# hanruihua/RDA-planner

Measured on NVIDIA H100. Metric: MPC solves/sec (T=30, 20 obs, 50 ADMM iters), higher is better.
Workload: dtype f32 state / f64 su-QP interior point

## Files before the change

### rda_planner_b200/csrc/rda_kernels.cu

```cuda
#include <cuda_runtime.h>
#include <stdio.h>
#include <stdlib.h>
#include <string.h>
#include <new>
#include "rda_hd.h"
#include "cell_solver.cuh"
#include "su_solver.cuh"
#include "cell_lean.cuh"
#include "cell_lean2.cuh"
#include "cell_disc_robot.cuh"

using namespace rda;

struct SmallLayout {
  int lam, mu, z, xi, zeta, dis, coef, pref, cur_s, cur_u, ref_s, misc, hs, su, wl, slow, total;
};

struct rda_handle {
  rda_config cfg;
  rda_tunables tun;
  RobotGeom rb;
  int B, T, N, E, R;
  int sms;
  float *lam, *mu, *z, *xi, *zeta, *dis, *coef, *pref, *cur_s, *cur_u, *ref_s, *ref_speed;
  float *resi_acc, *resi_pri, *resi_dual;
  int *status, *iters, *done, *counters, *worklist, *worklist2;
  char* su_ws;
  size_t su_ws_stride;
  int lean2;
  RobotAux ra;
  ObstacleGeom<4>* ogeo;
  unsigned char* feat;
  int* worklist0;
  float* rot;
  const float *obs_A, *obs_b;
  const int *obs_kind, *obs_count;
  int obs_tv;
  float iter_threshold;
  int launches;
  int began;
  cudaStream_t side[3];
  cudaEvent_t ev_fork, ev_join[3];
  int small_mode;
  int small_max, small_ok, small_bulk;
  SmallLayout small_L;
  float su_prune;
  int extra_min;
  int split_min;
  int parts;
};

#define RDA_CUDA(x) do { cudaError_t e_ = (x); if (e_ != cudaSuccess) return (int)e_; } while (0)

namespace {

struct WarpCtx {
  __device__ __forceinline__ int lane() const { return threadIdx.x & 31; }
  __device__ __forceinline__ int nlanes() const { return 32; }
  __device__ __forceinline__ void sync() const { __syncwarp(); }
  template <typename R> __device__ __forceinline__ R sum(R x) const {
    for (int o = 16; o > 0; o >>= 1) x += __shfl_xor_sync(0xffffffffu, x, o);
    return x;
  }
  template <typename R> __device__ __forceinline__ R min(R x) const {
    for (int o = 16; o > 0; o >>= 1) { R y = __shfl_xor_sync(0xffffffffu, x, o); x = y < x ? y : x; }
    return x;
  }
  template <typename R> __device__ __forceinline__ R max(R x) const {
    for (int o = 16; o > 0; o >>= 1) { R y = __shfl_xor_sync(0xffffffffu, x, o); x = y > x ? y : x; }
    return x;
  }
};

struct DevPtrs {
  float *lam, *mu, *z, *xi, *zeta, *dis, *coef, *pref, *cur_s, *cur_u, *ref_s, *ref_speed;
  float *resi_acc, *resi_pri, *resi_dual;
  int *status, *iters, *done, *counters, *worklist, *worklist2;
  int* wl_count;
  const ObstacleGeom<4>* ogeo;
  unsigned char* feat;
  int* worklist0;
  char* su_ws;
  size_t su_ws_stride;
  const float *obs_A, *obs_b;
  const int *obs_kind, *obs_count;
  int obs_tv;
  int B, T, N, E, R;
};

__global__ void k_begin(DevPtrs d, const float* nom_s, const float* nom_u, const float* ref_s,
                        const float* ref_speed) {
  const int T = d.T;
  const int per = 3 * (T + 1);
  const int total = d.B * per;
  for (int i = blockIdx.x * blockDim.x + threadIdx.x; i < total; i += gridDim.x * blockDim.x) {
    d.cur_s[i] = nom_s[i];
    d.ref_s[i] = ref_s[i];
    int b = i / per, r = i - b * per;
    if (r < 2 * T) d.cur_u[b * 2 * T + r] = nom_u[b * 2 * T + r];
    if (r == 0) {
      d.ref_speed[b] = ref_speed[b];
      d.done[b] = 0; d.iters[b] = 0; d.status[b] = 0;
      d.resi_acc[2 * b] = 0; d.resi_acc[2 * b + 1] = 0;
      d.resi_pri[b] = 0; d.resi_dual[b] = 0;
    }
  }
}

template <typename Real>
__device__ __forceinline__ void su_instance(const DevPtrs& d, const SuParams& P, int b, SuWork<Real>& W, WarpCtx& ctx) {
  const int T = P.T, N = P.N, NT = N * T;
  const int lane = ctx.lane();
  const float* cs = d.cur_s + (size_t)b * 3 * (T + 1);
  const float* cu = d.cur_u + (size_t)b * 2 * T;
  const float* rf = d.ref_s + (size_t)b * 3 * (T + 1);
  for (int i = lane; i < 3 * (T + 1); i += 32) {
    int r = i / (T + 1), t = i - r * (T + 1);
    W.lins[3 * t + r] = cs[i];
    W.ref[3 * t + r] = rf[i];
  }
  for (int i = lane; i < 2 * T; i += 32) {
    int r = i / T, t = i - r * T;
    W.linu[2 * t + r] = cu[i];
    W.pref[2 * t + r] = d.pref[(size_t)b * 2 * T + i];
  }
  for (int t = lane; t < T; t += 32) W.d[t] = d.dis[(size_t)b * T + t];
  float* cf = d.coef + (size_t)b * 5 * NT;
  W.hx = cf; W.hy = cf + NT; W.hc = cf + 2 * NT;
  W.vref = d.ref_speed[b];
  ctx.sync();
  int iters = 0;
  int st = su_solve<Real, WarpCtx>(P, W, ctx, cf + 3 * NT, cf + 4 * NT, &iters);
  ctx.sync();
  bool ok = st != 2;
// ... 2 lines not shown
      int r = i / (T + 1), t = i - r * (T + 1);
      float v = (float)W.s[3 * t + r];
      if (!isfinite(v)) ok = false;
    }
    for (int i = lane; i < 2 * T; i += 32) {
      int r = i / T, t = i - r * T;
      if (!isfinite((float)W.u[2 * t + r])) ok = false;
    }
    ok = ctx.min((int)ok) != 0;
  }
  if (ok) {
    float* ws = d.cur_s + (size_t)b * 3 * (T + 1);
    float* wu = d.cur_u + (size_t)b * 2 * T;
    for (int i = lane; i < 3 * (T + 1); i += 32) {
      int r = i / (T + 1), t = i - r * (T + 1);
      ws[i] = (float)W.s[3 * t + r];
    }
    for (int i = lane; i < 2 * T; i += 32) {
      int r = i / T, t = i - r * T;
      wu[i] = (float)W.u[2 * t + r];
    }
    for (int t = lane; t < T; t += 32) d.dis[(size_t)b * T + t] = (float)W.d[t];
  }
  if (lane == 0) {
    d.iters[b] += 1;
    int flag = 0;
    if (st == 1) flag |= RDA_ST_SU_NOT_CONVERGED;
    if (!ok) flag |= RDA_ST_SU_NONFINITE;
    if (flag) d.status[b] |= flag;
    atomicAdd(&d.counters[3], iters);
    atomicAdd(&d.counters[4], 1);
    if (W.restarts) atomicAdd(&d.counters[5], 1);
  }
}

template <typename Real>
__global__ void __launch_bounds__(32) k_su(DevPtrs d, SuParams P) {
  extern __shared__ __align__(16) char smem[];
  const int b = blockIdx.x;
  if (b >= d.B) return;
  if (d.done[b]) return;
  WarpCtx ctx;
  SuWork<Real> W;
  su_work_layout<Real>(P.T, P.N, &W, smem, false, d.su_ws + (size_t)b * d.su_ws_stride);
  su_instance<Real>(d, P, b, W, ctx);
}

struct CellIn {
  int b, o, t, kind;
  size_t cell;
  float px, py, cp, sp, dbar, zeta, xi0, xi1;
  const float *A, *bb;
};

__device__ __forceinline__ CellIn cell_load(const DevPtrs& d, long long idx) {
  const int T = d.T, N = d.N, E = d.E, NT = N * T;
  CellIn c;
  c.b = (int)(idx / NT);
  const int rem = (int)(idx - (long long)c.b * NT);
  c.o = rem / T; c.t = rem - c.o * T;
  const float* cs = d.cur_s + (size_t)c.b * 3 * (T + 1);
  c.px = cs[c.t + 1]; c.py = cs[(T + 1) + c.t + 1];
  sincosf(cs[2 * (T + 1) + c.t], &c.sp, &c.cp);
  c.dbar = d.dis[(size_t)c.b * T + c.t];
  c.cell = (size_t)c.b * NT + (size_t)c.o * T + c.t;
  c.zeta = d.zeta[c.cell];
  const float* xi = d.xi + (size_t)c.b * 2 * NT;
  c.xi0 = xi[(size_t)c.o * T + c.t]; c.xi1 = xi[NT + (size_t)c.o * T + c.t];
  const int tc = d.obs_tv ? (c.t + 1) : 0;
  const int Tc = d.obs_tv ? (T + 1) : 1;
  const size_t ob = ((size_t)c.b * N + c.o) * Tc + tc;
  c.A = d.obs_A + ob * E * 2;
  c.bb = d.obs_b + ob * E;
  c.kind = d.obs_kind[(size_t)c.b * N + c.o];
  return c;
}

__device__ __forceinline__ void cell_store(const DevPtrs& d, const CellIn& c, const CellOut<float>& out, float* hm2,
                                           float* dual) {
  const int T = d.T, N = d.N, E = d.E, R = d.R, NT = N * T;
  float* lam = d.lam + ((size_t)c.b * N + c.o) * E * T + c.t;
  float acc = 0.f;
  for (int i = 0; i < E; ++i) {
    float nv = out.lam[i];
    float df = nv - lam[(size_t)i * T];
    acc += df * df;
    lam[(size_t)i * T] = nv;
  }
  float* mu = d.mu + ((size_t)c.b * N + c.o) * R * T + c.t;
  for (int j = 0; j < R; ++j) {
    float nv = out.mu[j];
    float df = nv - mu[(size_t)j * T];
    acc += df * df;
    mu[(size_t)j * T] = nv;
  }
  float dz = out.z - d.z[c.cell];
  acc += dz * dz;
  d.z[c.cell] = out.z;
  *dual = acc;
  d.zeta[c.cell] = out.zeta_new;
  float* xi = d.xi + (size_t)c.b * 2 * NT;
  xi[(size_t)c.o * T + c.t] = out.xi0_new;
  xi[NT + (size_t)c.o * T + c.t] = out.xi1_new;
  *hm2 = out.hm0 * out.hm0 + out.hm1 * out.hm1;
  float* cf = d.coef + (size_t)c.b * 5 * NT + (size_t)c.o * T + c.t;
  cf[0] = out.ax;
  cf[NT] = out.ay;
  cf[2 * NT] = out.c0;
  cf[3 * NT] = out.gx;
  cf[4 * NT] = out.gy;
  if (c.o == 0) {
    d.pref[(size_t)c.b * 2 * T + c.t] = c.px;
    d.pref[(size_t)c.b * 2 * T + T + c.t] = c.py;
  }
}

template <int EC, int RC, bool LISTED>
__global__ void __launch_bounds__(128, (EC <= 4 ? 6 : 3)) k_cells_fast(DevPtrs d, RobotGeom rb, float theta) {
  const int T = d.T, N = d.N, E = d.E, R = d.R;
  const int NT = N * T;
  const long long total = LISTED ? (long long)d.wl_count[2] : (long long)d.B * NT;
  const int lane = threadIdx.x & 31;
  for (long long base = (long long)blockIdx.x * blockDim.x; base < total; base += (long long)gridDim.x * blockDim.x) {
    long long idx = base + threadIdx.x;
    bool live = idx < total;
    if (LISTED && live) idx = d.worklist0[idx];
    int b = live ? (int)(idx / NT) : -1;
    float dual = 0.f;
    bool need = false;
    if (live && (d.done[b] || d.obs_count[b] == 0)) live = false;
    if (live) {
      CellIn c = cell_load(d, idx);
      float Ar[2 * EC], br[EC], lamo[EC], muo[RC];
      if (EC == 4 && E == 4) {
        const float4 a0 = __ldg(reinterpret_cast<const float4*>(c.A));
        const float4 a1 = __ldg(reinterpret_cast<const float4*>(c.A) + 1);
        const float4 b0 = __ldg(reinterpret_cast<const float4*>(c.bb));
        Ar[0] = a0.x; Ar[1] = a0.y; Ar[2] = a0.z; Ar[3] = a0.w;
        Ar[(4) % (2 * EC)] = a1.x; Ar[(5) % (2 * EC)] = a1.y; Ar[(6) % (2 * EC)] = a1.z; Ar[(7) % (2 * EC)] = a1.w;
        br[0] = b0.x; br[1 % EC] = b0.y; br[2 % EC] = b0.z; br[3 % EC] = b0.w;
      } else {
#pragma unroll
        for (int i = 0; i < EC; ++i) {
          Ar[2 * i] = (i < E) ? __ldg(c.A + 2 * i) : 0.f;
          Ar[2 * i + 1] = (i < E) ? __ldg(c.A + 2 * i + 1) : 0.f;
          br[i] = (i < E) ? __ldg(c.bb + i) : 0.f;
        }
      }
      const float* lamp = d.lam + ((size_t)c.b * N + c.o) * E * T + c.t;
      const float* mup = d.mu + ((size_t)c.b * N + c.o) * R * T + c.t;
#pragma unroll
      for (int i = 0; i < EC; ++i) lamo[i] = (i < E) ? lamp[(size_t)i * T] : 0.f;
#pragma unroll
      for (int j = 0; j < RC; ++j) muo[j] = (j < R) ? mup[(size_t)j * T] : 0.f;
      const float zo = d.z[c.cell];
      LeanOut<EC, RC> o;
      const bool ok = cell_lean<EC, RC>(rb, c.kind, EC, Ar, br, c.px, c.py, c.cp, c.sp, c.dbar, c.zeta, c.xi0,
                                        c.xi1, theta, o);
      if (d.feat) d.feat[c.cell] = (unsigned char)(ok ? o.feat : 0);
      if (ok) {
        float* lam = d.lam + ((size_t)c.b * N + c.o) * E * T + c.t;
        float acc = 0.f;
#pragma unroll
        for (int i = 0; i < EC; ++i) {
          if (i < E) {
            const float df = o.lam[i] - lamo[i];
            acc += df * df;
            lam[(size_t)i * T] = o.lam[i];
          }
        }
        float* mu = d.mu + ((size_t)c.b * N + c.o) * R * T + c.t;
#pragma unroll
        for (int j = 0; j < RC; ++j) {
          if (j < R) {
            const float df = o.mu[j] - muo[j];
            acc += df * df;
            mu[(size_t)j * T] = o.mu[j];
          }
        }
        const float dz = o.z - zo;
        acc += dz * dz;
        d.z[c.cell] = o.z;
        dual = acc;
        d.zeta[c.cell] = o.zeta_new;
        float* cf = d.coef + (size_t)c.b * 5 * NT + (size_t)c.o * T + c.t;
        cf[0] = o.ax; cf[NT] = o.ay; cf[2 * NT] = o.c0; cf[3 * NT] = o.gx; cf[4 * NT] = o.gy;
        if (c.o == 0) {
          d.pref[(size_t)c.b * 2 * T + c.t] = c.px;
          d.pref[(size_t)c.b * 2 * T + T + c.t] = c.py;
        }
      } else {
        need = true;
      }
    }
    unsigned nm = __ballot_sync(0xffffffffu, need);
    if (nm) {
      int leader = __ffs(nm) - 1, pos = 0;
      if (lane == leader) pos = atomicAdd(&d.wl_count[0], __popc(nm));
      pos = __shfl_sync(0xffffffffu, pos, leader);
      if (need) d.worklist[pos + __popc(nm & ((1u << lane) - 1))] = (int)idx;
    }
    const bool solved = live && !need;
    if (LISTED) {
      if (solved) atomicAdd(&d.resi_acc[2 * b + 1], dual);
      unsigned fastl = __ballot_sync(0xffffffffu, solved);
      if (lane == 0 && fastl) atomicAdd(&d.counters[0], __popc(fastl));
      continue;
    }
    int b0 = __shfl_sync(0xffffffffu, b, 0);
    for (int pass = 0; pass < 2; ++pass) {
      bool mine = solved && ((pass == 0) ? (b == b0) : (b != b0));
      unsigned m = __ballot_sync(0xffffffffu, mine);
      if (m == 0) continue;
      float q = mine ? dual : 0.f;
      int leader = __ffs(m) - 1;
      int bl = __shfl_sync(0xffffffffu, b, leader);
      bool uniform = __all_sync(0xffffffffu, !mine || b == bl);
      if (uniform) {
        for (int o2 = 16; o2 > 0; o2 >>= 1) q += __shfl_xor_sync(0xffffffffu, q, o2);
        if (lane == leader) atomicAdd(&d.resi_acc[2 * bl + 1], q);
      } else if (mine) {
        atomicAdd(&d.resi_acc[2 * b + 1], q);
      }
    }
    unsigned fast = __ballot_sync(0xffffffffu, solved);
    if (lane == 0 && fast) atomicAdd(&d.counters[0], __popc(fast));
  }
}

__global__ void k_obstacle_geometry(DevPtrs d, ObstacleGeom<4>* og) {
  const int i = blockIdx.x * blockDim.x + threadIdx.x;
  if (i >= d.B * d.N) return;
  ObstacleGeom<4> g;
  if (d.obs_kind[i] == RDA_OBS_POLYGON && d.E <= 4) obstacle_geometry<4>(d.E, d.obs_A + (size_t)i * d.E * 2, d.obs_b + (size_t)i * d.E, g);
  else { obstacle_geometry<4>(0, nullptr, nullptr, g); }
  og[i] = g;
}

__global__ void k_heading(DevPtrs d, float* rot) {
  const int i = blockIdx.x * blockDim.x + threadIdx.x;
  const int T = d.T;
  if (i >= d.B * T) return;
  const int b = i / T, t = i - b * T;
  float sp, cp;
  sincosf(d.cur_s[(size_t)b * 3 * (T + 1) + 2 * (T + 1) + t], &sp, &cp);
  rot[(size_t)b * 2 * T + t] = cp;
  rot[(size_t)b * 2 * T + T + t] = sp;
}

__global__ void __launch_bounds__(128, 6) k_cells_coh(DevPtrs d, RobotGeom rb, RobotAux ra, const float* __restrict__ rot,
                                                      float theta, float invT, int tiles) {
  constexpr int EC = 4, RC = 4;
  const int T = d.T, N = d.N, E = d.E, R = d.R, NT = N * T;
  const int b = blockIdx.x / tiles;
  if (d.done[b] || d.obs_count[b] == 0) return;
  const int rem = (blockIdx.x - b * tiles) * blockDim.x + threadIdx.x;
  const int lane = threadIdx.x & 31;
  const bool live = rem < NT;
  float dual = 0.f;
  bool need = false, solved = false;
  if (live) {
    int o = (int)(((float)rem + 0.5f) * invT);
    int t = rem - o * T;
    if (t < 0) { --o; t += T; } else if (t >= T) { ++o; t -= T; }
    const size_t ib = (size_t)b;
    const float* cs = d.cur_s + ib * 3 * (T + 1);
    const float* xi = d.xi + ib * 2 * NT;
    float* lamb = d.lam + ib * N * E * T;
    float* mub = d.mu + ib * N * R * T;
    float* zb = d.z + ib * NT;
    float* zetab = d.zeta + ib * NT;
    unsigned char* featb = d.feat + ib * NT;
    const float xi0 = xi[rem], xi1 = xi[NT + rem];
    const int f = featb[rem];
    int nf = -1;
    if (xi0 == 0.f && xi1 == 0.f && (f & RDA_FEAT_VALID)) {
      const float px = cs[t + 1], py = cs[(T + 1) + t + 1];
      const float cp = rot[ib * 2 * T + t], sp = rot[ib * 2 * T + T + t];
      const float dbar = d.dis[ib * T + t], zeta = zetab[rem];
      const int lo = o * E * T + t, mo = o * R * T + t;
      float lamo[EC], muo[RC];
#pragma unroll
      for (int i = 0; i < EC; ++i) lamo[i] = (i < E) ? lamb[lo + i * T] : 0.f;
#pragma unroll
      for (int j = 0; j < RC; ++j) muo[j] = (j < R) ? mub[mo + j * T] : 0.f;
      const float zo = zb[rem];
      const ObstacleGeom<4>& og = d.ogeo[ib * N + o];
      LeanOut<EC, RC> r;
      nf = cell_lean2<EC, RC>(rb, ra, og, f, px, py, cp, sp, dbar, zeta, theta, r);
      if (nf >= 0) {
        float acc = 0.f;
#pragma unroll
        for (int i = 0; i < EC; ++i) {
          if (i < E) { const float df = r.lam[i] - lamo[i]; acc += df * df; lamb[lo + i * T] = r.lam[i]; }
        }
#pragma unroll
        for (int j = 0; j < RC; ++j) {
          if (j < R) { const float df = r.mu[j] - muo[j]; acc += df * df; mub[mo + j * T] = r.mu[j]; }
        }
        const float dz = r.z - zo;
        acc += dz * dz;
        zb[rem] = r.z;
        dual = acc;
        zetab[rem] = r.zeta_new;
        float* cf = d.coef + ib * 5 * NT + rem;
        cf[0] = r.ax; cf[NT] = r.ay; cf[2 * NT] = r.c0; cf[3 * NT] = r.gx; cf[4 * NT] = r.gy;
        if (o == 0) {
          d.pref[ib * 2 * T + t] = px;
          d.pref[ib * 2 * T + T + t] = py;
        }
        if (nf != f) featb[rem] = (unsigned char)nf;
        solved = true;
      }
    }
    need = nf < 0;
  }
  const unsigned nm = __ballot_sync(0xffffffffu, need);
  if (nm) {
    const int leader = __ffs(nm) - 1;
    int pos = 0;
    if (lane == leader) pos = atomicAdd(&d.wl_count[2], __popc(nm));
    pos = __shfl_sync(0xffffffffu, pos, leader);
    if (need) d.worklist0[pos + __popc(nm & ((1u << lane) - 1))] = b * NT + rem;
  }
  const unsigned fast = __ballot_sync(0xffffffffu, solved);
  if (fast) {
    float q = dual;
    for (int o2 = 16; o2 > 0; o2 >>= 1) q += __shfl_xor_sync(0xffffffffu, q, o2);
    if (lane == 0) { atomicAdd(&d.resi_acc[2 * b + 1], q); atomicAdd(&d.counters[0], __popc(fast)); }
  }
}

struct RowsLocal { float A[2 * RDA_MAX_EDGE], b[RDA_MAX_EDGE]; };
__device__ __forceinline__ void rows_preload(const DevPtrs& d, const CellIn& c, RowsLocal& r) {
  if (d.E == 4) {
    const float4 a0 = __ldg(reinterpret_cast<const float4*>(c.A));
    const float4 a1 = __ldg(reinterpret_cast<const float4*>(c.A) + 1);
    const float4 b0 = __ldg(reinterpret_cast<const float4*>(c.bb));
    r.A[0] = a0.x; r.A[1] = a0.y; r.A[2] = a0.z; r.A[3] = a0.w; r.A[4] = a1.x; r.A[5] = a1.y; r.A[6] = a1.z; r.A[7] = a1.w;
    r.b[0] = b0.x; r.b[1] = b0.y; r.b[2] = b0.z; r.b[3] = b0.w;
  } else {
#pragma unroll
    for (int i = 0; i < RDA_MAX_EDGE; ++i) {
      const bool in = i < d.E;
      r.A[2 * i] = in ? __ldg(c.A + 2 * i) : 0.f;
      r.A[2 * i + 1] = in ? __ldg(c.A + 2 * i + 1) : 0.f;
      r.b[i] = in ? __ldg(c.bb + i) : 0.f;
    }
  }
}

__global__ void __launch_bounds__(128) k_cells_mid(DevPtrs d, RobotGeom rb, float ro2, float theta) {
  const int count = d.wl_count[0];
  const int lane = threadIdx.x & 31;
  for (int base = blockIdx.x * blockDim.x; base < count; base += gridDim.x * blockDim.x) {
    const int wi = base + threadIdx.x;
    const bool live = wi < count;
    bool need = false;
    long long idx = 0;
    if (live) {
      idx = d.worklist[wi];
      CellIn c = cell_load(d, idx);
      RowsLocal rows;
      rows_preload(d, c, rows);
      CellWork<float> w;
      cell_front<float, false>(rb, c.kind, d.E, rows.A, rows.b, c.px, c.py, c.cp, c.sp, c.dbar, c.zeta, c.xi0, c.xi1, ro2, w);
      if (w.have) {
        CellOut<float> out;
        cell_back<float>(rb, w, c.zeta, theta, out);
        float hm2 = 0.f, dual = 0.f;
        cell_store(d, c, out, &hm2, &dual);
        atomicAdd(&d.resi_acc[2 * c.b], hm2);
        atomicAdd(&d.resi_acc[2 * c.b + 1], dual);
      } else {
        need = true;
      }
    }
    unsigned m = __ballot_sync(0xffffffffu, need);
    if (m) {
      int leader = __ffs(m) - 1, pos = 0;
      if (lane == leader) pos = atomicAdd(&d.wl_count[1], __popc(m));
      pos = __shfl_sync(0xffffffffu, pos, leader);
      if (need) d.worklist2[pos + __popc(m & ((1u << lane) - 1))] = (int)idx;
    }
    unsigned solved = __ballot_sync(0xffffffffu, live && !need);
    if (lane == 0 && solved) atomicAdd(&d.counters[0], __popc(solved));
  }
}

__global__ void __launch_bounds__(128) k_cells_dr(DevPtrs d, RobotGeom rb, float ro2, float theta) {
  const int NT = d.N * d.T;
  const long long total = (long long)d.B * NT;
  const int lane = threadIdx.x & 31;
  for (long long base = (long long)blockIdx.x * blockDim.x; base < total; base += (long long)gridDim.x * blockDim.x) {
    const long long idx = base + threadIdx.x;
    bool live = idx < total;
    const int b = live ? (int)(idx / NT) : -1;
    if (live && (d.done[b] || d.obs_count[b] == 0)) live = false;
    bool need = false;
    if (live) {
      CellIn c = cell_load(d, idx);
      CellWork<float> w;
      cell_front_dr<float>(rb, c.kind, d.E, c.A, c.bb, c.px, c.py, c.cp, c.sp, c.dbar, c.zeta, c.xi0, c.xi1, ro2, w, false);
      if (w.have) {
        CellOut<float> out;
        cell_back_dr<float>(rb, w, c.zeta, theta, out);
        float hm2 = 0.f, dual = 0.f;
        cell_store(d, c, out, &hm2, &dual);
        atomicAdd(&d.resi_acc[2 * c.b], hm2);
        atomicAdd(&d.resi_acc[2 * c.b + 1], dual);
      } else {
        need = true;
      }
    }
    const unsigned m = __ballot_sync(0xffffffffu, need);
    if (m) {
      int leader = __ffs(m) - 1, pos = 0;
      if (lane == leader) pos = atomicAdd(&d.wl_count[1], __popc(m));
      pos = __shfl_sync(0xffffffffu, pos, leader);
      if (need) d.worklist2[pos + __popc(m & ((1u << lane) - 1))] = (int)idx;
    }
    const unsigned solved = __ballot_sync(0xffffffffu, live && !need);
    if (lane == 0 && solved) atomicAdd(&d.counters[0], __popc(solved));
  }
}

__global__ void __launch_bounds__(128) k_cells_dr_mid(DevPtrs d, RobotGeom rb, float ro2, float theta) {
  const int count = d.wl_count[1];
  const int lane = threadIdx.x & 31;
  for (int base = blockIdx.x * blockDim.x; base < count; base += gridDim.x * blockDim.x) {
    const int wi = base + threadIdx.x;
    bool need = false;
    int idx = 0;
    if (wi < count) {
      idx = d.worklist2[wi];
      CellIn c = cell_load(d, idx);
      CellWork<float> w;
// ... 13 lines not shown
    const unsigned m = __ballot_sync(0xffffffffu, need);
    if (m) {
      int leader = __ffs(m) - 1, pos = 0;
      if (lane == leader) pos = atomicAdd(&d.wl_count[4], __popc(m));
      pos = __shfl_sync(0xffffffffu, pos, leader);
      if (need) d.worklist[pos + __popc(m & ((1u << lane) - 1))] = idx;
    }
  }
}

constexpr int COOP_WARPS = 4;

__global__ void __launch_bounds__(32 * COOP_WARPS) k_cells_dr_slow_coop(DevPtrs d, RobotGeom rb, float ro2, float theta) {
  __shared__ DiscSlowStore store[COOP_WARPS];
  const int count = d.wl_count[4];
  const int warp = threadIdx.x >> 5, lane = threadIdx.x & 31;
  DiscSlowStore& S = store[warp];
  WarpCtx ctx;
  for (int wi = blockIdx.x * COOP_WARPS + warp; wi < count; wi += gridDim.x * COOP_WARPS) {
    const long long idx = d.worklist[wi];
    CellIn c;
    CellWork<float> w;
    w.have = false;
    if (lane == 0) {
      c = cell_load(d, idx);
      cell_front_dr<float>(rb, c.kind, d.E, c.A, c.bb, c.px, c.py, c.cp, c.sp, c.dbar, c.zeta, c.xi0, c.xi1, ro2, w, false);
    }
    const int have = __shfl_sync(0xffffffffu, (int)w.have, 0);
    if (!have) {
      __syncwarp();
      cell_slow_dr<float, WarpCtx>(rb, w, S, ctx);
      __syncwarp();
    }
    if (lane == 0) {
      CellOut<float> out;
      cell_back_dr<float>(rb, w, c.zeta, theta, out);
      float hm2 = 0.f, dual = 0.f;
      if (out.path == CELL_FAILED) {
        dual = INFINITY;
        atomicOr(&d.status[c.b], RDA_ST_CELL_FALLBACK);
      } else {
        cell_store(d, c, out, &hm2, &dual);
      }
      atomicAdd(&d.resi_acc[2 * c.b], hm2);
      atomicAdd(&d.resi_acc[2 * c.b + 1], dual);
      atomicAdd(&d.counters[out.path == CELL_FAILED ? 2 : 1], 1);
    }
    __syncwarp();
  }
}

__global__ void __launch_bounds__(128) k_cells_extra(DevPtrs d, RobotGeom rb, float ro2, float theta) {
  const int count = d.wl_count[1];
  const int lane = threadIdx.x & 31;
  for (int base = blockIdx.x * blockDim.x; base < count; base += gridDim.x * blockDim.x) {
    const int wi = base + threadIdx.x;
    bool need = false;
    int idx = 0;
    if (wi < count) {
      idx = d.worklist2[wi];
      CellIn c = cell_load(d, idx);
      RowsLocal rows;
      rows_preload(d, c, rows);
      CellWork<float> w;
      cell_front<float, false, true>(rb, c.kind, d.E, rows.A, rows.b, c.px, c.py, c.cp, c.sp, c.dbar, c.zeta, c.xi0, c.xi1, ro2, w);
      if (w.have) {
        CellOut<float> out;
        cell_back<float>(rb, w, c.zeta, theta, out);
        float hm2 = 0.f, dual = 0.f;
        cell_store(d, c, out, &hm2, &dual);
        atomicAdd(&d.resi_acc[2 * c.b], hm2);
        atomicAdd(&d.resi_acc[2 * c.b + 1], dual);
        atomicAdd(&d.counters[1], 1);
      } else {
        need = true;
      }
    }
    const unsigned m = __ballot_sync(0xffffffffu, need);
    if (m) {
      int leader = __ffs(m) - 1, pos = 0;
      if (lane == leader) pos = atomicAdd(&d.wl_count[4], __popc(m));
      pos = __shfl_sync(0xffffffffu, pos, leader);
      if (need) d.worklist[pos + __popc(m & ((1u << lane) - 1))] = idx;
    }
  }
}

__global__ void __launch_bounds__(32 * COOP_WARPS) k_cells_slow_coop(DevPtrs d, RobotGeom rb, float ro2, float theta, int from_extra) {
  __shared__ CellSlowStore store[COOP_WARPS];
  const int count = from_extra ? d.wl_count[4] : d.wl_count[1];
  const int* list = from_extra ? d.worklist : d.worklist2;
  const int warp = threadIdx.x >> 5, lane = threadIdx.x & 31;
  CellSlowStore& S = store[warp];
  WarpCtx ctx;
  for (int wi = blockIdx.x * COOP_WARPS + warp; wi < count; wi += gridDim.x * COOP_WARPS) {
    const long long idx = list[wi];
    CellIn c;
    CellWork<float> w;
    w.have = false;
    if (lane == 0) {
      c = cell_load(d, idx);
      cell_front<float, false, true>(rb, c.kind, d.E, c.A, c.bb, c.px, c.py, c.cp, c.sp, c.dbar, c.zeta, c.xi0, c.xi1, ro2, w);
    }
    const int have = __shfl_sync(0xffffffffu, (int)w.have, 0);
    if (!have) {
      __syncwarp();
      cell_slow<float, WarpCtx>(rb, w, S, ctx);
      __syncwarp();
    }
    if (lane == 0) {
      CellOut<float> out;
      cell_back<float>(rb, w, c.zeta, theta, out);
      float hm2 = 0.f, dual = 0.f;
      if (out.path == CELL_FAILED) {
        dual = INFINITY;
        atomicOr(&d.status[c.b], RDA_ST_CELL_FALLBACK);
      } else {
        cell_store(d, c, out, &hm2, &dual);
      }
      atomicAdd(&d.resi_acc[2 * c.b], hm2);
      atomicAdd(&d.resi_acc[2 * c.b + 1], dual);
      atomicAdd(&d.counters[out.path == CELL_FAILED ? 2 : 1], 1);
    }
    __syncwarp();
  }
}

__device__ __forceinline__ void finalize_instance(const DevPtrs& d, const RobotGeom& rb, float thr, int b) {
  const int T = d.T, N = d.N, NT = N * T, R = d.R;
  float pri = 0.f, dual = 0.f;
  if (N > 0 && d.obs_count[b] != 0) {
    pri = sqrtf(d.resi_acc[2 * b]);
    dual = d.resi_acc[2 * b + 1] / (float)N;
  } else if (N > 0) {
    int o = N - 1;
    float* cf = d.coef + (size_t)b * 5 * NT + (size_t)o * T;
    for (int t = 0; t < T; ++t) {
      const float* mu = d.mu + ((size_t)b * N + o) * R * T + t;
      float muh = 0.f;
      for (int j = 0; j < R; ++j) muh += mu[(size_t)j * T] * rb.h[j];
      size_t cell = (size_t)b * NT + (size_t)o * T + t;
      cf[t] = 0.f; cf[NT + t] = 0.f;
      cf[2 * NT + t] = -muh - d.z[cell] + d.zeta[cell];
    }
  }
  d.resi_acc[2 * b] = 0.f; d.resi_acc[2 * b + 1] = 0.f;
  d.resi_pri[b] = pri; d.resi_dual[b] = dual;
  if (dual < thr && pri < thr) { d.done[b] = 1; d.status[b] |= RDA_ST_EARLY_STOP; }
}

__global__ void k_finalize(DevPtrs d, RobotGeom rb, float thr) {
  int b = blockIdx.x * blockDim.x + threadIdx.x;
  if (b == 0) { d.wl_count[0] = 0; d.wl_count[1] = 0; d.wl_count[2] = 0; d.wl_count[3] = 0; d.wl_count[4] = 0; }
  if (b >= d.B) return;
  if (d.done[b]) return;
  finalize_instance(d, rb, thr, b);
}

static SmallLayout small_layout(int T, int N, int E, int R, size_t su_bytes, size_t su_gbytes) {
  SmallLayout L;
  size_t o = 0;
  auto take = [&](size_t bytes) { o = (o + 15) & ~(size_t)15; size_t r = o; o += bytes; return (int)r; };
  const size_t NT = (size_t)N * T;
  L.lam = take(4 * N * E * T); L.mu = take(4 * N * R * T); L.z = take(4 * NT); L.xi = take(8 * NT); L.zeta = take(4 * NT);
  L.dis = take(4 * T); L.coef = take(20 * NT); L.pref = take(8 * T); L.cur_s = take(12 * (T + 1)); L.cur_u = take(8 * T);
  L.ref_s = take(12 * (T + 1)); L.misc = take(128); L.hs = take(su_gbytes); L.su = take(su_bytes);
  L.wl = take(4 * (NT + 1)); L.slow = take(4 * sizeof(CellSlowStore));
  L.total = (int)((o + 15) & ~(size_t)15);
  return L;
}

// ... 189 lines not shown
    ((float*)out.resi_pri)[b] = misc[2]; ((float*)out.resi_dual)[b] = misc[3];
    ((int*)out.status)[b] = ds.status[0]; ((int*)out.iters)[b] = ds.iters[0];
  }
}

__global__ void k_finish(DevPtrs d, rda_outputs o) {
  const int T = d.T;
  const int per = 3 * (T + 1);
  const int total = d.B * per;
  for (int i = blockIdx.x * blockDim.x + threadIdx.x; i < total; i += gridDim.x * blockDim.x) {
    o.s_opt[i] = d.cur_s[i];
    int b = i / per, r = i - b * per;
    if (r < 2 * T) o.u_opt[b * 2 * T + r] = d.cur_u[b * 2 * T + r];
    if (r == 0) {
      o.resi_pri[b] = d.resi_pri[b]; o.resi_dual[b] = d.resi_dual[b];
      o.status[b] = d.status[b]; o.iters[b] = d.iters[b];
    }
  }
}

__global__ void k_reset(DevPtrs d, RobotGeom rb) {
  const int T = d.T, N = d.N, NT = N * T, R = d.R;
  const long long total = (long long)d.B * NT;
  for (long long idx = (long long)blockIdx.x * blockDim.x + threadIdx.x; idx < total; idx += (long long)gridDim.x * blockDim.x) {
    int b = (int)(idx / NT);
    int rem = (int)(idx - (long long)b * NT);
    int o = rem / T, t = rem - o * T;
    const float* mu = d.mu + ((size_t)b * N + o) * R * T + t;
    float muh = 0.f;
    for (int j = 0; j < R; ++j) muh += mu[(size_t)j * T] * rb.h[j];
    float* cf = d.coef + (size_t)b * 5 * NT + rem;
    cf[0] = 0.f; cf[NT] = 0.f;
    cf[2 * NT] = -muh - d.z[idx] + d.zeta[idx];
  }
}

__global__ void k_fill(float* p, float v, size_t n) {
  for (size_t i = (size_t)blockIdx.x * blockDim.x + threadIdx.x; i < n; i += (size_t)gridDim.x * blockDim.x) p[i] = v;
}

DevPtrs dev_ptrs(const rda_handle* h, int b0, int nb, int part) {
  DevPtrs d;
  const size_t o = (size_t)b0, T = h->T, N = h->N, E = h->E, R = h->R, NT = N * T;
  const size_t Tc = h->obs_tv ? T + 1 : 1;
  d.lam = h->lam + o * N * E * T; d.mu = h->mu + o * N * R * T; d.z = h->z + o * NT; d.xi = h->xi + o * 2 * NT;
  d.zeta = h->zeta + o * NT; d.dis = h->dis + o * T; d.coef = h->coef + o * 5 * NT; d.pref = h->pref + o * 2 * T;
  d.cur_s = h->cur_s + o * 3 * (T + 1); d.cur_u = h->cur_u + o * 2 * T; d.ref_s = h->ref_s + o * 3 * (T + 1);
  d.ref_speed = h->ref_speed + o; d.resi_acc = h->resi_acc + 2 * o; d.resi_pri = h->resi_pri + o;
  d.resi_dual = h->resi_dual + o;
  d.status = h->status + o; d.iters = h->iters + o; d.done = h->done + o;
  d.counters = h->counters; d.wl_count = h->counters + 8 + 8 * part;
  d.ogeo = h->ogeo ? h->ogeo + o * N : nullptr;
  d.feat = h->feat ? h->feat + o * NT : nullptr;
  d.worklist0 = h->worklist0 ? h->worklist0 + o * NT : nullptr;
  d.worklist = h->worklist + o * NT; d.worklist2 = h->worklist2 + o * NT;
  d.su_ws = h->su_ws + o * h->su_ws_stride; d.su_ws_stride = h->su_ws_stride;
  d.obs_A = h->obs_A ? h->obs_A + o * N * Tc * E * 2 : nullptr;
  d.obs_b = h->obs_b ? h->obs_b + o * N * Tc * E : nullptr;
  d.obs_kind = h->obs_kind ? h->obs_kind + o * N : nullptr;
  d.obs_count = h->obs_count ? h->obs_count + o : nullptr;
  d.obs_tv = h->obs_tv;
  d.B = nb; d.T = h->T; d.N = h->N; d.E = h->E; d.R = h->R;
  return d;
}

DevPtrs dev_ptrs(const rda_handle* h) { return dev_ptrs(h, 0, h->B, 0); }

SuParams su_params(const rda_handle* h) {
  SuParams P;
  P.T = h->T; P.N = h->N; P.dynamics = h->cfg.dynamics; P.accelerated = h->cfg.accelerated;
  P.dt = h->cfg.step_time; P.L = h->cfg.wheelbase;
  P.umax[0] = h->cfg.max_speed[0]; P.umax[1] = h->cfg.max_speed[1];
  P.ab[0] = h->cfg.acce_bound[0]; P.ab[1] = h->cfg.acce_bound[1];
  P.ws = h->cfg.ws; P.wu = h->cfg.wu;
  P.slack_gain = h->tun.slack_gain; P.dmin = h->tun.min_sd; P.dmax = h->tun.max_sd;
  P.ro1 = h->tun.ro1; P.ro2 = h->tun.ro2;
  P.max_iter = 40;
  P.mu0 = 1.0f;
  P.prune = h->su_prune;
  return P;
}

int grid_for(long long n, int block, int sms) {
  long long g = (n + block - 1) / block;
  const long long cap = 16LL * sms;
  if (g > cap) g = cap;
  if (g < 1) g = 1;
  return (int)g;
}

}

extern "C" {

const char* rda_version(void) { return "rda_b200 0.1 (sm_90a)"; }

int rda_create(const rda_config* cfg, const rda_tunables* tun, rda_handle** out) {
  if (!cfg || !tun || !out) return RDA_E_ARG;
  if (cfg->batch < 1 || cfg->receding < 1 || cfg->max_obs_num < 0) return RDA_E_ARG;
  if (cfg->max_edge_num < 3 || cfg->max_edge_num > RDA_MAX_EDGE) return RDA_E_UNSUPPORTED;
  if (cfg->dynamics < 0 || cfg->dynamics > 2) return RDA_E_ARG;
  rda_handle* h = new (std::nothrow) rda_handle();
  if (!h) return RDA_E_NOMEM;
  memset(h, 0, sizeof(*h));
  h->cfg = *cfg; h->tun = *tun;
  int rc = robot_geom_from_halfspaces(cfg->G, cfg->h, cfg->robot_edges, &h->rb, cfg->robot_cone);
  if (rc) { delete h; return rc; }
  h->B = cfg->batch; h->T = cfg->receding; h->N = cfg->max_obs_num; h->E = cfg->max_edge_num;
  h->R = cfg->robot_edges;
  const size_t B = h->B, T = h->T, N = h->N, E = h->E, R = h->R, NT = N * T;
  {
    size_t g = 0;
    const size_t sm = cfg->su_fp64 ? su_work_bytes<double>((int)T, (int)N, false, &g) : su_work_bytes<float>((int)T, (int)N, false, &g);
    if (sm > 227 * 1024) { delete h; return RDA_E_UNSUPPORTED; }
    h->su_ws_stride = (g + 127) & ~(size_t)127;
  }
  int dev = 0;
  cudaError_t e = cudaGetDevice(&dev);
  if (e == cudaSuccess) e = cudaDeviceGetAttribute(&h->sms, cudaDevAttrMultiProcessorCount, dev);
  if (e != cudaSuccess) { delete h; return (int)e; }
  auto alloc = [&](float** p, size_t n) { if (e == cudaSuccess) e = cudaMalloc((void**)p, (n ? n : 1) * sizeof(float)); };
  alloc(&h->lam, B * N * E * T); alloc(&h->mu, B * N * R * T); alloc(&h->z, B * NT);
  alloc(&h->xi, B * 2 * NT); alloc(&h->zeta, B * NT); alloc(&h->dis, B * T);
  alloc(&h->coef, B * 5 * NT); alloc(&h->pref, B * 2 * T); alloc(&h->cur_s, B * 3 * (T + 1));
  alloc(&h->cur_u, B * 2 * T); alloc(&h->ref_s, B * 3 * (T + 1)); alloc(&h->ref_speed, B);
  alloc(&h->resi_acc, B * 2); alloc(&h->resi_pri, B); alloc(&h->resi_dual, B);
  alloc((float**)&h->status, B); alloc((float**)&h->iters, B); alloc((float**)&h->done, B);
  alloc((float**)&h->counters, 64);
  alloc((float**)&h->worklist, B * NT);
  alloc((float**)&h->worklist2, B * NT);
  alloc((float**)&h->su_ws, B * (h->su_ws_stride / 4));
  if (e != cudaSuccess) { rda_destroy(h); return (int)e; }
  e = cfg->su_fp64 ? cudaFuncSetAttribute(k_su<double>, cudaFuncAttributeMaxDynamicSharedMemorySize, 227 * 1024)
                   : cudaFuncSetAttribute(k_su<float>, cudaFuncAttributeMaxDynamicSharedMemorySize, 227 * 1024);
  if (e != cudaSuccess) { rda_destroy(h); return (int)e; }
  e = cudaEventCreateWithFlags(&h->ev_fork, cudaEventDisableTiming);
  for (int p = 0; p < 3; ++p) {
    if (e == cudaSuccess) e = cudaStreamCreateWithFlags(&h->side[p], cudaStreamNonBlocking);
    if (e == cudaSuccess) e = cudaEventCreateWithFlags(&h->ev_join[p], cudaEventDisableTiming);
  }
  if (e != cudaSuccess) { rda_destroy(h); return (int)e; }
  h->lean2 = h->B >= 8192 && h->E <= 4 && h->R <= 4 && h->N > 0 && !h->rb.disc;
  if (const char* l2 = getenv("RDA_B200_LEAN2")) h->lean2 = atoi(l2) != 0 && h->E <= 4 && h->R <= 4 && h->N > 0 && !h->rb.disc;
  if (h->lean2) {
    robot_aux_from_geom(h->rb, &h->ra);
    e = cudaMalloc((void**)&h->ogeo, B * N * sizeof(ObstacleGeom<4>));
    if (e == cudaSuccess) e = cudaMalloc((void**)&h->feat, B * NT ? B * NT : 1);
    if (e == cudaSuccess) e = cudaMalloc((void**)&h->worklist0, (B * NT ? B * NT : 1) * sizeof(int));
    if (e == cudaSuccess) e = cudaMalloc((void**)&h->rot, B * 2 * T * sizeof(float));
    if (e != cudaSuccess) { rda_destroy(h); return (int)e; }
  }
  h->split_min = 2048;
  h->parts = 2;
  h->su_prune = 0.5f;
  {
    size_t g = 0;
    const size_t sub = cfg->su_fp64 ? su_work_bytes<double>((int)T, (int)N, false, &g) : su_work_bytes<float>((int)T, (int)N, false, &g);
    h->small_L = small_layout((int)T, (int)N, (int)E, (int)R, sub, g);
    h->small_ok = h->small_L.total <= 200 * 1024 && !h->rb.disc;
    h->small_mode = -1; h->small_max = 2 * h->sms;
    h->small_bulk = (N > 0) && ((N * E * T) % 4 == 0) && ((N * R * T) % 4 == 0) && ((N * T) % 4 == 0);
    if (const char* v = getenv("RDA_B200_SMALL_BULK")) { if (atoi(v) == 0) h->small_bulk = 0; }
    if (const char* v = getenv("RDA_B200_SMALL")) { int x = atoi(v); if (x >= -1 && x <= 1) h->small_mode = x; }
    if (const char* v = getenv("RDA_B200_SMALL_MAX")) { int x = atoi(v); if (x >= 1) h->small_max = x; }
    if (h->small_ok) {
      if (cfg->su_fp64) e = cudaFuncSetAttribute(k_admm_small<double>, cudaFuncAttributeMaxDynamicSharedMemorySize, h->small_L.total);
      else e = cudaFuncSetAttribute(k_admm_small<float>, cudaFuncAttributeMaxDynamicSharedMemorySize, h->small_L.total);
      if (e != cudaSuccess) { rda_destroy(h); return (int)e; }
    }
  }
  if (const char* v = getenv("RDA_B200_SU_PRUNE")) { float x = (float)atof(v); if (x >= 0.f) h->su_prune = x; }
  h->extra_min = 3000;
  if (const char* v = getenv("RDA_B200_EXTRA_MIN")) { int x = atoi(v); if (x >= 1) h->extra_min = x; }
  if (const char* sm = getenv("RDA_B200_SPLIT_MIN")) { int v = atoi(sm); if (v >= 2) h->split_min = v; }
  if (const char* sp = getenv("RDA_B200_SPLIT_PARTS")) { int v = atoi(sp); if (v >= 1 && v <= 4) h->parts = v; }
  rc = rda_cold_start(h, nullptr);
  if (rc) { rda_destroy(h); return rc; }
  e = cudaDeviceSynchronize();
  if (e != cudaSuccess) { rda_destroy(h); return (int)e; }
  *out = h;
  return 0;
}

int rda_destroy(rda_handle* h) {
  if (!h) return RDA_E_ARG;
  float* bufs[] = {h->lam, h->mu, h->z, h->xi, h->zeta, h->dis, h->coef, h->pref, h->cur_s, h->cur_u,
                   h->ref_s, h->ref_speed, h->resi_acc, h->resi_pri, h->resi_dual, (float*)h->status,
                   (float*)h->iters, (float*)h->done, (float*)h->counters, (float*)h->worklist, (float*)h->worklist2, (float*)h->su_ws};
  for (float* p : bufs) if (p) cudaFree(p);
  if (h->ogeo) cudaFree(h->ogeo);
  if (h->feat) cudaFree(h->feat);
  if (h->worklist0) cudaFree(h->worklist0);
  if (h->rot) cudaFree(h->rot);
  if (h->ev_fork) cudaEventDestroy(h->ev_fork);
  for (int p = 0; p < 3; ++p) {
    if (h->ev_join[p]) cudaEventDestroy(h->ev_join[p]);
    if (h->side[p]) cudaStreamDestroy(h->side[p]);
  }
  delete h;
  return 0;
}

int rda_set_tunables(rda_handle* h, const rda_tunables* tun) {
  if (!h || !tun) return RDA_E_ARG;
  h->tun = *tun;
  return 0;
}

int rda_get_tunables(const rda_handle* h, rda_tunables* tun) {
  if (!h || !tun) return RDA_E_ARG;
  *tun = h->tun;
  return 0;
}

int rda_cold_start(rda_handle* h, void* stream) {
  if (!h) return RDA_E_ARG;
  cudaStream_t s = (cudaStream_t)stream;
  const size_t B = h->B, T = h->T, N = h->N, E = h->E, R = h->R, NT = N * T;
  RDA_CUDA(cudaMemsetAsync(h->lam, 0, B * N * E * T * 4, s));
  RDA_CUDA(cudaMemsetAsync(h->mu, 0, B * N * R * T * 4, s));
  RDA_CUDA(cudaMemsetAsync(h->z, 0, B * NT * 4, s));
  RDA_CUDA(cudaMemsetAsync(h->xi, 0, B * 2 * NT * 4, s));
  RDA_CUDA(cudaMemsetAsync(h->zeta, 0, B * NT * 4, s));
  RDA_CUDA(cudaMemsetAsync(h->coef, 0, B * 5 * NT * 4, s));
  RDA_CUDA(cudaMemsetAsync(h->pref, 0, B * 2 * T * 4, s));
  RDA_CUDA(cudaMemsetAsync(h->cur_s, 0, B * 3 * (T + 1) * 4, s));
  RDA_CUDA(cudaMemsetAsync(h->cur_u, 0, B * 2 * T * 4, s));
  RDA_CUDA(cudaMemsetAsync(h->resi_acc, 0, B * 2 * 4, s));
  RDA_CUDA(cudaMemsetAsync(h->resi_pri, 0, B * 4, s));
  RDA_CUDA(cudaMemsetAsync(h->resi_dual, 0, B * 4, s));
  RDA_CUDA(cudaMemsetAsync(h->status, 0, B * 4, s));
  RDA_CUDA(cudaMemsetAsync(h->iters, 0, B * 4, s));
  RDA_CUDA(cudaMemsetAsync(h->done, 0, B * 4, s));
  RDA_CUDA(cudaMemsetAsync(h->counters, 0, 64 * 4, s));
  if (h->feat) RDA_CUDA(cudaMemsetAsync(h->feat, 0, B * NT, s));
  k_fill<<<grid_for((long long)(B * T), 256, h->sms), 256, 0, s>>>(h->dis, 1.0f, B * T);
  RDA_CUDA(cudaGetLastError());
  h->launches = 1;
  return 0;
}

int rda_reset(rda_handle* h, void* stream) {
  if (!h) return RDA_E_ARG;
  if (h->N == 0) return 0;
  DevPtrs d = dev_ptrs(h);
// ... 236 lines not shown
```

Baseline: 25010.

## Replace index worklists with packed 80-byte cell records carrying state and duals

Worklists between the cell kernels (lean2 to fast, fast to slow, slow to extra, extra to coop) now hold full per-cell records. Each record carries position, rotation, dbar, zeta, xi and the previous lam/mu/z, so downstream kernels skip the scattered gathers and recomputation in cell_load and use the stored previous duals for the dual residual. The cost is wider worklist writes (80 bytes instead of 4 per entry), the lean2 kernel now loading duals for every cell, and two large record buffers allocated per handle.

```diff
diff --git a/rda_planner_b200/csrc/rda_kernels.cu b/rda_planner_b200/csrc/rda_kernels.cu
--- a/rda_planner_b200/csrc/rda_kernels.cu
+++ b/rda_planner_b200/csrc/rda_kernels.cu
@@ -16,6 +16,14 @@
   int lam, mu, z, xi, zeta, dis, coef, pref, cur_s, cur_u, ref_s, misc, hs, su, wl, slow, total;
 };
 
+struct __align__(16) CellRec {
+  int cell, kind;
+  float px, py, cp, sp, dbar, zeta, xi0, xi1;
+  float lam[4], mu[4], z;
+  int pad_;
+};
+static_assert(sizeof(CellRec) == 80, "CellRec: five 16-byte words");
+
 struct rda_handle {
   rda_config cfg;
   rda_tunables tun;
@@ -25,13 +33,13 @@
   float *lam, *mu, *z, *xi, *zeta, *dis, *coef, *pref, *cur_s, *cur_u, *ref_s, *ref_speed;
   float *resi_acc, *resi_pri, *resi_dual;
   int *status, *iters, *done, *counters, *worklist, *worklist2;
+  CellRec *rec_a, *rec_b;
   char* su_ws;
   size_t su_ws_stride;
   int lean2;
   RobotAux ra;
   ObstacleGeom<4>* ogeo;
   unsigned char* feat;
-  int* worklist0;
   float* rot;
   const float *obs_A, *obs_b;
   const int *obs_kind, *obs_count;
@@ -79,7 +87,7 @@
   int* wl_count;
   const ObstacleGeom<4>* ogeo;
   unsigned char* feat;
-  int* worklist0;
+  CellRec *rec_a, *rec_b;
   char* su_ws;
   size_t su_ws_stride;
   const float *obs_A, *obs_b;
@@ -188,6 +196,14 @@
   float px, py, cp, sp, dbar, zeta, xi0, xi1;
   const float *A, *bb;
 };
+
+__device__ __forceinline__ void cell_rows(const DevPtrs& d, CellIn& c) {
+  const int tc = d.obs_tv ? (c.t + 1) : 0;
+  const int Tc = d.obs_tv ? (d.T + 1) : 1;
+  const size_t ob = ((size_t)c.b * d.N + c.o) * Tc + tc;
+  c.A = d.obs_A + ob * d.E * 2;
+  c.bb = d.obs_b + ob * d.E;
+}
 
 __device__ __forceinline__ CellIn cell_load(const DevPtrs& d, long long idx) {
   const int T = d.T, N = d.N, E = d.E, NT = N * T;
@@ -212,25 +228,75 @@
   return c;
 }
 
+__device__ __forceinline__ bool rec_duals(const DevPtrs& d) { return d.E <= 4 && d.R <= 4; }
+
+__device__ __forceinline__ CellRec cell_rec(const CellIn& c) {
+  CellRec r;
+  r.cell = (int)c.cell; r.kind = c.kind;
+  r.px = c.px; r.py = c.py; r.cp = c.cp; r.sp = c.sp; r.dbar = c.dbar; r.zeta = c.zeta; r.xi0 = c.xi0; r.xi1 = c.xi1;
+  r.pad_ = 0;
+  return r;
+}
+
+__device__ __forceinline__ CellIn cell_from_rec(const DevPtrs& d, const CellRec& r) {
+  const int T = d.T, NT = d.N * T;
+  CellIn c;
+  c.cell = (size_t)r.cell;
+  c.b = r.cell / NT;
+  const int rem = r.cell - c.b * NT;
+  c.o = rem / T; c.t = rem - c.o * T;
+  c.kind = r.kind;
+  c.px = r.px; c.py = r.py; c.cp = r.cp; c.sp = r.sp; c.dbar = r.dbar; c.zeta = r.zeta; c.xi0 = r.xi0; c.xi1 = r.xi1;
+  cell_rows(d, c);
+  return c;
+}
+
+__device__ __forceinline__ CellRec cell_rec_load(const DevPtrs& d, long long idx) {
+  const CellIn c = cell_load(d, idx);
+  CellRec r = cell_rec(c);
+  const int T = d.T, N = d.N, E = d.E, R = d.R;
+  const float* lam = d.lam + ((size_t)c.b * N + c.o) * E * T + c.t;
+  const float* mu = d.mu + ((size_t)c.b * N + c.o) * R * T + c.t;
+#pragma unroll
+  for (int i = 0; i < 4; ++i) {
+    r.lam[i] = i < E ? lam[(size_t)i * T] : 0.f;
+    r.mu[i] = i < R ? mu[(size_t)i * T] : 0.f;
+  }
+  r.z = d.z[c.cell];
+  return r;
+}
+
+__device__ __forceinline__ CellRec* rec_slot(bool need, CellRec* list, int* count) {
+  const int lane = threadIdx.x & 31;
+  const unsigned m = __ballot_sync(0xffffffffu, need);
+  if (!m) return nullptr;
+  const int leader = __ffs(m) - 1;
+  int pos = 0;
+  if (lane == leader) pos = atomicAdd(count, __popc(m));
+  pos = __shfl_sync(0xffffffffu, pos, leader);
+  return need ? list + pos + __popc(m & ((1u << lane) - 1)) : nullptr;
+}
+
 __device__ __forceinline__ void cell_store(const DevPtrs& d, const CellIn& c, const CellOut<float>& out, float* hm2,
-                                           float* dual) {
+                                           float* dual, const CellRec* prev = nullptr) {
   const int T = d.T, N = d.N, E = d.E, R = d.R, NT = N * T;
+  const bool pr = prev != nullptr && rec_duals(d);
   float* lam = d.lam + ((size_t)c.b * N + c.o) * E * T + c.t;
   float acc = 0.f;
   for (int i = 0; i < E; ++i) {
     float nv = out.lam[i];
-    float df = nv - lam[(size_t)i * T];
+    float df = nv - (pr ? prev->lam[i] : lam[(size_t)i * T]);
     acc += df * df;
     lam[(size_t)i * T] = nv;
   }
   float* mu = d.mu + ((size_t)c.b * N + c.o) * R * T + c.t;
   for (int j = 0; j < R; ++j) {
     float nv = out.mu[j];
-    float df = nv - mu[(size_t)j * T];
+    float df = nv - (pr ? prev->mu[j] : mu[(size_t)j * T]);
     acc += df * df;
     mu[(size_t)j * T] = nv;
   }
-  float dz = out.z - d.z[c.cell];
+  float dz = out.z - (prev != nullptr ? prev->z : d.z[c.cell]);
   acc += dz * dz;
   d.z[c.cell] = out.z;
   *dual = acc;
@@ -258,15 +324,17 @@
   const long long total = LISTED ? (long long)d.wl_count[2] : (long long)d.B * NT;
   const int lane = threadIdx.x & 31;
   for (long long base = (long long)blockIdx.x * blockDim.x; base < total; base += (long long)gridDim.x * blockDim.x) {
-    long long idx = base + threadIdx.x;
+    const long long wi = base + threadIdx.x;
+    long long idx = wi;
     bool live = idx < total;
-    if (LISTED && live) idx = d.worklist0[idx];
+    CellRec rec;
+    if (LISTED && live) { rec = d.rec_a[wi]; idx = rec.cell; }
     int b = live ? (int)(idx / NT) : -1;
     float dual = 0.f;
     bool need = false;
-    if (live && (d.done[b] || d.obs_count[b] == 0)) live = false;
+    if (!LISTED && live && (d.done[b] || d.obs_count[b] == 0)) live = false;
     if (live) {
-      CellIn c = cell_load(d, idx);
+      CellIn c = LISTED ? cell_from_rec(d, rec) : cell_load(d, idx);
       float Ar[2 * EC], br[EC], lamo[EC], muo[RC];
       if (EC == 4 && E == 4) {
         const float4 a0 = __ldg(reinterpret_cast<const float4*>(c.A));
@@ -283,13 +351,22 @@
           br[i] = (i < E) ? __ldg(c.bb + i) : 0.f;
         }
       }
-      const float* lamp = d.lam + ((size_t)c.b * N + c.o) * E * T + c.t;
-      const float* mup = d.mu + ((size_t)c.b * N + c.o) * R * T + c.t;
+      float zo;
+      if (LISTED) {
 #pragma unroll
-      for (int i = 0; i < EC; ++i) lamo[i] = (i < E) ? lamp[(size_t)i * T] : 0.f;
+        for (int i = 0; i < EC; ++i) lamo[i] = (i < E) ? rec.lam[i % 4] : 0.f;
 #pragma unroll
-      for (int j = 0; j < RC; ++j) muo[j] = (j < R) ? mup[(size_t)j * T] : 0.f;
-      const float zo = d.z[c.cell];
+        for (int j = 0; j < RC; ++j) muo[j] = (j < R) ? rec.mu[j % 4] : 0.f;
+        zo = rec.z;
+      } else {
+        const float* lamp = d.lam + ((size_t)c.b * N + c.o) * E * T + c.t;
+        const float* mup = d.mu + ((size_t)c.b * N + c.o) * R * T + c.t;
+#pragma unroll
+        for (int i = 0; i < EC; ++i) lamo[i] = (i < E) ? lamp[(size_t)i * T] : 0.f;
+#pragma unroll
+        for (int j = 0; j < RC; ++j) muo[j] = (j < R) ? mup[(size_t)j * T] : 0.f;
+        zo = d.z[c.cell];
+      }
       LeanOut<EC, RC> o;
       const bool ok = cell_lean<EC, RC>(rb, c.kind, EC, Ar, br, c.px, c.py, c.cp, c.sp, c.dbar, c.zeta, c.xi0,
                                         c.xi1, theta, o);
@@ -329,13 +406,7 @@
         need = true;
       }
     }
-    unsigned nm = __ballot_sync(0xffffffffu, need);
-    if (nm) {
-      int leader = __ffs(nm) - 1, pos = 0;
-      if (lane == leader) pos = atomicAdd(&d.wl_count[0], __popc(nm));
-      pos = __shfl_sync(0xffffffffu, pos, leader);
-      if (need) d.worklist[pos + __popc(nm & ((1u << lane) - 1))] = (int)idx;
-    }
+    if (CellRec* s = rec_slot(need, d.rec_b, &d.wl_count[0])) *s = LISTED ? d.rec_a[wi] : cell_rec_load(d, idx);
     const bool solved = live && !need;
     if (LISTED) {
       if (solved) atomicAdd(&d.resi_acc[2 * b + 1], dual);
@@ -395,6 +466,7 @@
   const bool live = rem < NT;
   float dual = 0.f;
   bool need = false, solved = false;
+  CellRec rec;
   if (live) {
     int o = (int)(((float)rem + 0.5f) * invT);
     int t = rem - o * T;
@@ -409,18 +481,18 @@
     unsigned char* featb = d.feat + ib * NT;
     const float xi0 = xi[rem], xi1 = xi[NT + rem];
     const int f = featb[rem];
+    const float px = cs[t + 1], py = cs[(T + 1) + t + 1];
+    const float cp = rot[ib * 2 * T + t], sp = rot[ib * 2 * T + T + t];
+    const float dbar = d.dis[ib * T + t], zeta = zetab[rem];
+    const int lo = o * E * T + t, mo = o * R * T + t;
+    float lamo[EC], muo[RC];
+#pragma unroll
+    for (int i = 0; i < EC; ++i) lamo[i] = (i < E) ? lamb[lo + i * T] : 0.f;
+#pragma unroll
+    for (int j = 0; j < RC; ++j) muo[j] = (j < R) ? mub[mo + j * T] : 0.f;
+    const float zo = zb[rem];
     int nf = -1;
     if (xi0 == 0.f && xi1 == 0.f && (f & RDA_FEAT_VALID)) {
-      const float px = cs[t + 1], py = cs[(T + 1) + t + 1];
-      const float cp = rot[ib * 2 * T + t], sp = rot[ib * 2 * T + T + t];
-      const float dbar = d.dis[ib * T + t], zeta = zetab[rem];
-      const int lo = o * E * T + t, mo = o * R * T + t;
-      float lamo[EC], muo[RC];
-#pragma unroll
-      for (int i = 0; i < EC; ++i) lamo[i] = (i < E) ? lamb[lo + i * T] : 0.f;
-#pragma unroll
-      for (int j = 0; j < RC; ++j) muo[j] = (j < R) ? mub[mo + j * T] : 0.f;
-      const float zo = zb[rem];
       const ObstacleGeom<4>& og = d.ogeo[ib * N + o];
       LeanOut<EC, RC> r;
       nf = cell_lean2<EC, RC>(rb, ra, og, f, px, py, cp, sp, dbar, zeta, theta, r);
@@ -450,15 +522,15 @@
       }
     }
     need = nf < 0;
-  }
-  const unsigned nm = __ballot_sync(0xffffffffu, need);
-  if (nm) {
-    const int leader = __ffs(nm) - 1;
-    int pos = 0;
-    if (lane == leader) pos = atomicAdd(&d.wl_count[2], __popc(nm));
-    pos = __shfl_sync(0xffffffffu, pos, leader);
-    if (need) d.worklist0[pos + __popc(nm & ((1u << lane) - 1))] = b * NT + rem;
-  }
+    if (need) {
+      rec.cell = b * NT + rem; rec.kind = d.obs_kind[ib * N + o];
+      rec.px = px; rec.py = py; rec.cp = cp; rec.sp = sp; rec.dbar = dbar; rec.zeta = zeta; rec.xi0 = xi0; rec.xi1 = xi1;
+#pragma unroll
+      for (int i = 0; i < 4; ++i) { rec.lam[i] = lamo[i]; rec.mu[i] = muo[i]; }
+      rec.z = zo; rec.pad_ = 0;
+    }
+  }
+  if (CellRec* s = rec_slot(need, d.rec_a, &d.wl_count[2])) *s = rec;
   const unsigned fast = __ballot_sync(0xffffffffu, solved);
   if (fast) {
     float q = dual;
@@ -493,10 +565,8 @@
     const int wi = base + threadIdx.x;
     const bool live = wi < count;
     bool need = false;
-    long long idx = 0;
     if (live) {
-      idx = d.worklist[wi];
-      CellIn c = cell_load(d, idx);
+      CellIn c = cell_from_rec(d, d.rec_b[wi]);
       RowsLocal rows;
       rows_preload(d, c, rows);
       CellWork<float> w;
@@ -505,20 +575,14 @@
         CellOut<float> out;
         cell_back<float>(rb, w, c.zeta, theta, out);
         float hm2 = 0.f, dual = 0.f;
-        cell_store(d, c, out, &hm2, &dual);
+        cell_store(d, c, out, &hm2, &dual, d.rec_b + wi);
         atomicAdd(&d.resi_acc[2 * c.b], hm2);
         atomicAdd(&d.resi_acc[2 * c.b + 1], dual);
       } else {
         need = true;
       }
     }
-    unsigned m = __ballot_sync(0xffffffffu, need);
-    if (m) {
-      int leader = __ffs(m) - 1, pos = 0;
-      if (lane == leader) pos = atomicAdd(&d.wl_count[1], __popc(m));
-      pos = __shfl_sync(0xffffffffu, pos, leader);
-      if (need) d.worklist2[pos + __popc(m & ((1u << lane) - 1))] = (int)idx;
-    }
+    if (CellRec* s = rec_slot(need, d.rec_a, &d.wl_count[1])) *s = d.rec_b[wi];
     unsigned solved = __ballot_sync(0xffffffffu, live && !need);
     if (lane == 0 && solved) atomicAdd(&d.counters[0], __popc(solved));
   }
@@ -638,14 +702,11 @@
 
 __global__ void __launch_bounds__(128) k_cells_extra(DevPtrs d, RobotGeom rb, float ro2, float theta) {
   const int count = d.wl_count[1];
-  const int lane = threadIdx.x & 31;
   for (int base = blockIdx.x * blockDim.x; base < count; base += gridDim.x * blockDim.x) {
     const int wi = base + threadIdx.x;
     bool need = false;
-    int idx = 0;
     if (wi < count) {
-      idx = d.worklist2[wi];
-      CellIn c = cell_load(d, idx);
+      CellIn c = cell_from_rec(d, d.rec_a[wi]);
       RowsLocal rows;
       rows_preload(d, c, rows);
       CellWork<float> w;
@@ -654,7 +715,7 @@
         CellOut<float> out;
         cell_back<float>(rb, w, c.zeta, theta, out);
         float hm2 = 0.f, dual = 0.f;
-        cell_store(d, c, out, &hm2, &dual);
+        cell_store(d, c, out, &hm2, &dual, d.rec_a + wi);
         atomicAdd(&d.resi_acc[2 * c.b], hm2);
         atomicAdd(&d.resi_acc[2 * c.b + 1], dual);
         atomicAdd(&d.counters[1], 1);
@@ -662,30 +723,23 @@
         need = true;
       }
     }
-    const unsigned m = __ballot_sync(0xffffffffu, need);
-    if (m) {
-      int leader = __ffs(m) - 1, pos = 0;
-      if (lane == leader) pos = atomicAdd(&d.wl_count[4], __popc(m));
-      pos = __shfl_sync(0xffffffffu, pos, leader);
-      if (need) d.worklist[pos + __popc(m & ((1u << lane) - 1))] = idx;
-    }
+    if (CellRec* s = rec_slot(need, d.rec_b, &d.wl_count[4])) *s = d.rec_a[wi];
   }
 }
 
 __global__ void __launch_bounds__(32 * COOP_WARPS) k_cells_slow_coop(DevPtrs d, RobotGeom rb, float ro2, float theta, int from_extra) {
   __shared__ CellSlowStore store[COOP_WARPS];
   const int count = from_extra ? d.wl_count[4] : d.wl_count[1];
-  const int* list = from_extra ? d.worklist : d.worklist2;
+  const CellRec* list = from_extra ? d.rec_b : d.rec_a;
   const int warp = threadIdx.x >> 5, lane = threadIdx.x & 31;
   CellSlowStore& S = store[warp];
   WarpCtx ctx;
   for (int wi = blockIdx.x * COOP_WARPS + warp; wi < count; wi += gridDim.x * COOP_WARPS) {
-    const long long idx = list[wi];
     CellIn c;
     CellWork<float> w;
     w.have = false;
     if (lane == 0) {
-      c = cell_load(d, idx);
+      c = cell_from_rec(d, list[wi]);
       cell_front<float, false, true>(rb, c.kind, d.E, c.A, c.bb, c.px, c.py, c.cp, c.sp, c.dbar, c.zeta, c.xi0, c.xi1, ro2, w);
     }
     const int have = __shfl_sync(0xffffffffu, (int)w.have, 0);
@@ -702,7 +756,7 @@
         dual = INFINITY;
         atomicOr(&d.status[c.b], RDA_ST_CELL_FALLBACK);
       } else {
-        cell_store(d, c, out, &hm2, &dual);
+        cell_store(d, c, out, &hm2, &dual, list + wi);
       }
       atomicAdd(&d.resi_acc[2 * c.b], hm2);
       atomicAdd(&d.resi_acc[2 * c.b + 1], dual);
@@ -998,7 +1052,8 @@
   d.counters = h->counters; d.wl_count = h->counters + 8 + 8 * part;
   d.ogeo = h->ogeo ? h->ogeo + o * N : nullptr;
   d.feat = h->feat ? h->feat + o * NT : nullptr;
-  d.worklist0 = h->worklist0 ? h->worklist0 + o * NT : nullptr;
+  d.rec_a = h->rec_a ? h->rec_a + o * NT : nullptr;
+  d.rec_b = h->rec_b ? h->rec_b + o * NT : nullptr;
   d.worklist = h->worklist + o * NT; d.worklist2 = h->worklist2 + o * NT;
   d.su_ws = h->su_ws + o * h->su_ws_stride; d.su_ws_stride = h->su_ws_stride;
   d.obs_A = h->obs_A ? h->obs_A + o * N * Tc * E * 2 : nullptr;
@@ -1075,6 +1130,10 @@
   alloc((float**)&h->counters, 64);
   alloc((float**)&h->worklist, B * NT);
   alloc((float**)&h->worklist2, B * NT);
+  if (!h->rb.disc) {
+    alloc((float**)&h->rec_a, B * NT * (sizeof(CellRec) / 4));
+    alloc((float**)&h->rec_b, B * NT * (sizeof(CellRec) / 4));
+  }
   alloc((float**)&h->su_ws, B * (h->su_ws_stride / 4));
   if (e != cudaSuccess) { rda_destroy(h); return (int)e; }
   e = cfg->su_fp64 ? cudaFuncSetAttribute(k_su<double>, cudaFuncAttributeMaxDynamicSharedMemorySize, 227 * 1024)
@@ -1092,7 +1151,6 @@
     robot_aux_from_geom(h->rb, &h->ra);
     e = cudaMalloc((void**)&h->ogeo, B * N * sizeof(ObstacleGeom<4>));
     if (e == cudaSuccess) e = cudaMalloc((void**)&h->feat, B * NT ? B * NT : 1);
-    if (e == cudaSuccess) e = cudaMalloc((void**)&h->worklist0, (B * NT ? B * NT : 1) * sizeof(int));
     if (e == cudaSuccess) e = cudaMalloc((void**)&h->rot, B * 2 * T * sizeof(float));
     if (e != cudaSuccess) { rda_destroy(h); return (int)e; }
   }
@@ -1136,7 +1194,8 @@
   for (float* p : bufs) if (p) cudaFree(p);
   if (h->ogeo) cudaFree(h->ogeo);
   if (h->feat) cudaFree(h->feat);
-  if (h->worklist0) cudaFree(h->worklist0);
+  if (h->rec_a) cudaFree(h->rec_a);
+  if (h->rec_b) cudaFree(h->rec_b);
   if (h->rot) cudaFree(h->rot);
   if (h->ev_fork) cudaEventDestroy(h->ev_fork);
   for (int p = 0; p < 3; ++p) {
```

New measurement: 27150 (median of 6 runs). 1.09x the previous value.
